# pananananas/MVD

Hardware: AMD Instinct MI355X
Metric: UNet forward-passes/sec @512x512 SD2.1+MV adapter (higher is better)
Workload: dtype bf16; 1 GPU; cfg4: configs[3]/[4]: 8 objects x 4 target views per GPU (32 pairs), camera FiLM + cross-view adapter; pairs_per_gpu=32, global_pairs=32, latent=64x64x4, image=512x512, forward=cold, hip_graph=False, q2_statistics=replica-local, parallelism=dp1 (pairs sharded by object), weights=synthetic seeded, SD2.1 shapes (865.9M UNet x2 + 99.2M adapter + 19.1M camera), encoder_weights=distinct

## Files before the change

### include/mvd_hip.h

```cpp
#ifndef MVD_HIP_H
#define MVD_HIP_H
#include <stddef.h>
#include <stdint.h>

#ifdef __cplusplus
extern "C" {
#endif

#define MVD_MAX_LEVELS 4

typedef struct {
  int in_channels;
  int out_channels;
  int num_levels;
  int block_out_channels[MVD_MAX_LEVELS];
  int num_heads[MVD_MAX_LEVELS];
  int layers_per_block;
  int cross_attention_dim;
  int norm_num_groups;
  float norm_eps;
  int cam_output_dim;
  int cam_hidden_dim;
  int simple_cam_encoder;
  float cam_modulation_strength;
// ... 66 lines not shown
                  int ld_rowvec, int rows_per_batch, const void* res, float alpha, int geglu, void* out, int out_f32,
                  int m, int n, int force_cfg, int splitk, float* splitk_ws ,
                  void* stream);
int mvd_op_ln_linear(const void* x, int k, const void* w_folded, const float* c1, const float* c2, float eps, int geglu,
                     void* out, int m, int n, void* stream);
int mvd_op_linear_xs(const void* x, int ldx, const void* w_packed, int m, int k, int units, int geglu, int ln, float ln_eps,
                     const void* res, int ldres, void* out, int ldo, int csplit, void* stream);
int mvd_op_conv3x3_ws(const void* x, int batch, int h, int w, int c, const void* w_packed, const float* bias, const float* rowvec,
                      int ld_rowvec, const void* res, const void* sc, const void* sc2, int sc_c1, int sc_c2, void* out, int n,
                      int variant, void* stream);
int mvd_op_conv3x3(const void* x, int batch, int in_h, int in_w, int cin, int stride, int upsample, int asym_pad, const void* w,
                   const float* bias, const float* rowvec, int ld_rowvec, const void* res, const void* sc, const void* sc2,
                   int sc_c1, int sc_c2, void* out, int cout, int force_cfg, int splitk, float* splitk_ws, void* stream);
int mvd_op_conv3x3_up4(const void* x, int batch, int in_h, int in_w, int cin, const void* w4, const float* bias, void* out, int cout,
                       int force_cfg, void* stream);
int mvd_op_attention(const void* q, const void* k, const void* v, void* o, int batch, int heads, int nq, int nk, int ldq,
                     int ldk, int ldv, int ldo, float scale, void* stream);
int64_t mvd_op_attention_split_ws_bytes(int batch, int heads, int nq, int nsplit);
int mvd_op_attention_split(const void* q, const void* k, const void* v, void* o, int batch, int heads, int nq, int nk, int ldq,
                           int ldk, int ldv, int ldo, int nsplit, void* ws, void* stream);
int mvd_op_groupnorm(const void* x0, const void* x1, int c0, int c1, int batch, int hw, int groups, float eps,
                     const float* gamma, const float* beta, int silu, void* y, float* ws, void* stream);
int mvd_op_layernorm(const void* x, int rows, int c, float eps, const float* gamma, const float* beta, void* y,
                     void* stream);
int mvd_op_refnorm(const void* x, int batch, int hw, int c, void* y, void* stream);
int mvd_op_film(const void* x, int batch, int hw, int c, const float* scale, const float* shift, void* y, void* stream);
int mvd_op_conv_in(const void* x, int batch, int h, int w, int cin, const float* wt, const float* bias, int cout, void* y,
                   void* stream);
int mvd_op_conv_out(const void* x, int batch, int h, int w, int c, const void* wt, const float* bias, int cout, float* y,
                    void* stream);
// ... 154 lines not shown
```

### mvd_amd/_lib.py

```python
from __future__ import annotations

import ctypes as C
import enum
import os

HERE = os.path.dirname(os.path.abspath(__file__))
LIB_PATH = os.environ.get("MVD_HIP_LIB") or os.path.join(HERE, "libmvd_hip.so")

MVD_MAX_LEVELS = 4
MVD_USE_CAMERA, MVD_USE_IMAGE, MVD_REUSE_REF, MVD_KEEP_FEATURES = 1, 2, 4, 8


class MvdError(RuntimeError):
    pass


class DebugFlag(enum.IntFlag):
    NO_SM_LN_FOLD = 1
    SM_NO_SPLITK = 2
    NO_SM = 4
    NO_SPLIT_KV = 8
    ONE_STREAM = 16
    SINGLE_STREAM_POLICY = 32
    SIDE_DEFAULT_PRIORITY = 64
# ... 105 lines not shown
    "mvd_op_layernorm": (C.c_int, [C.c_void_p, C.c_int, C.c_int, C.c_float, C.c_void_p, C.c_void_p, C.c_void_p, C.c_void_p]),
    "mvd_op_refnorm": (C.c_int, [C.c_void_p, C.c_int, C.c_int, C.c_int, C.c_void_p, C.c_void_p]),
    "mvd_op_film": (C.c_int, [C.c_void_p, C.c_int, C.c_int, C.c_int, C.c_void_p, C.c_void_p, C.c_void_p, C.c_void_p]),
    "mvd_op_conv_in": (C.c_int, [C.c_void_p, C.c_int, C.c_int, C.c_int, C.c_int, C.c_void_p, C.c_void_p, C.c_int, C.c_void_p, C.c_void_p]),
    "mvd_op_conv_out": (C.c_int, [C.c_void_p, C.c_int, C.c_int, C.c_int, C.c_int, C.c_void_p, C.c_void_p, C.c_int, C.c_void_p, C.c_void_p]),
    "mvd_op_nchw_to_nhwc": (C.c_int, [C.c_void_p, C.c_int, C.c_int, C.c_int, C.c_void_p, C.c_void_p, C.c_void_p, C.c_void_p]),
    "mvd_op_nhwc_to_nchw": (C.c_int, [C.c_void_p, C.c_int, C.c_int, C.c_int, C.c_void_p, C.c_void_p]),
    "mvd_op_f32_to_bf16": (C.c_int, [C.c_void_p, C.c_int64, C.c_void_p, C.c_void_p]),
    "mvd_op_skinny_linear": (C.c_int, [C.c_void_p, C.c_int, C.c_int, C.c_int, C.c_void_p, C.c_int, C.c_void_p, C.c_int, C.c_int,
                                        C.c_void_p, C.c_int, C.c_void_p]),
    "mvd_gemm_num_configs": (C.c_int, []),
    "mvd_debug_last_gemm_plan": (C.c_int, [C.POINTER(C.c_int)]),
    "mvd_debug_up4_launches": (C.c_long, []),
    "mvd_op_conv3x3_up4": (C.c_int, [C.c_void_p, C.c_int, C.c_int, C.c_int, C.c_int, C.c_void_p, C.c_void_p, C.c_void_p, C.c_int, C.c_int,
                                     C.c_void_p]),
    "mvd_debug_last_gemm_nowait": (C.c_int, []),
    "mvd_debug_last_attention_plan": (C.c_int, [C.POINTER(C.c_int)]),
    "mvd_debug_pick_splitk": (C.c_int, [C.c_int, C.c_int, C.c_int, C.c_int]),
    "mvd_debug_pick_splitk_conv": (C.c_int, [C.c_int, C.c_int, C.c_int]),
    "mvd_gemm_sm_num_tiles": (C.c_int, []),
    "mvd_debug_set_attention_nw": (C.c_int, [C.c_int]),
    "mvd_debug_set_flags": (C.c_int, [C.c_int]),
    "mvd_op_ddpm_step": (C.c_int, [C.c_void_p, C.c_void_p, C.c_void_p, C.c_float, C.c_float, C.c_float, C.c_float,
                                   C.c_float, C.c_void_p, C.c_int64, C.c_void_p]),
    "mvd_op_cfg_combine": (C.c_int, [C.c_void_p, C.c_float, C.c_void_p, C.c_int64, C.c_void_p]),
    "mvd_op_sampler_step": (C.c_int, [C.c_void_p, C.c_int, C.c_float, C.c_void_p, C.c_void_p, C.c_void_p, C.c_float, C.c_float,
                                      C.c_float, C.c_float, C.c_float, C.c_float, C.c_void_p, C.c_void_p, C.c_int64, C.c_void_p]),
    "mvd_op_add_noise": (C.c_int, [C.c_void_p, C.c_void_p, C.c_void_p, C.c_void_p, C.c_void_p, C.c_int, C.c_void_p, C.c_void_p, C.c_int,
                                   C.c_int64, C.c_void_p]),
    "mvd_op_noise_loss_ws_bytes": (C.c_int64, [C.c_int, C.c_int64]),
# ... 91 lines not shown
```

### mvd_amd/csrc/engine.hip

```cpp
#include <math.h>
#include <stdio.h>
#include <stdlib.h>
#include <string.h>

#include <string>
#include <unordered_map>
#include <vector>

#include "host_util.h"

int mvd_launch_silu_to_bf16(const float* x, int64_t n, bf16_t* y, hipStream_t s);

static int g_debug_flags = 0;
extern "C" int mvd_debug_set_flags(int flags) { g_debug_flags = flags; return 0; }
int mvd_debug_flags() { return g_debug_flags; }

namespace {

struct FeatureInfo { std::string name; int level; int C; int heads; std::string key;  };
constexpr int MVD_REF_ONLY_INTERNAL = 1 << 30;

}

struct mvd_engine {
// ... 310 lines not shown
        g_debug_flags = saved;
        g_ws_ptrs[0] = (const char*)x.p; g_ws_lens[0] = (size_t)x.rows() * x.C * 2;
        g_ws_ptrs[1] = (const char*)sc0; g_ws_lens[1] = (size_t)out.rows() * scc0 * 2;
        g_ws_ptrs[2] = (const char*)sc1; g_ws_lens[2] = (size_t)out.rows() * scc1 * 2;
        g_ws_ptrs[3] = (const char*)out.p; g_ws_lens[3] = (size_t)out.rows() * out.C * 2;
        ws_check_launch(slot, set, nowait, out.p, chk.p, (long)out.rows() * out.C, s);
      }
      e->tmp.off = mark;
    }
#endif
    return r ? r : 1;
  }

  int conv3(const Act& x, int stride, int ups, const bf16_t* w, const float* bias, const float* rowvec, int ld_rowvec,
            const bf16_t* res, const bf16_t* sc0, const bf16_t* sc1, int scc0, int scc1, Act& out, const std::string& ws = std::string(),
            const std::string& w4 = std::string()) {
    if (!ws.empty() && stride == 1) {
      const int r = try_ws(x, ups, ws, bias, rowvec, ld_rowvec, res, sc0, sc1, scc0, scc1, out);
      if (r) return r < 0 ? r : 0;
    }
    MvdGemmArgs g = gemm_conv3(x.p, x.H, x.W, x.C, stride, ups, 0, sc0, sc1, scc0, scc1, w, bias, out.B, out.H, out.W, out.C, out.p);
    g.rowvec = rowvec; g.ld_rowvec = ld_rowvec; g.res = res;
    if (!w4.empty() && !dry && !err && ups == 1 && stride == 1 && !sc0 && !res && !rowvec && !(g_debug_flags & MVD_DBG_NO_UP4) && has(w4)) {
      int t_ = 0, n_ = 0, s_ = 1, S = 1, fc = -1;
      if (!(sm_enabled() && mvd_gemm_sm_plan(g, &t_, &n_, &s_))) {
        tiled_plan(g, S, fc);
        MvdGemmArgs u = g;
        u.splitk = 1;
        if (S == 1 && (fc >= 0 ? fc : mvd_gemm_pick_config(u)) == 7 && mvd_gemm_pp_applicable(u)) {
          gemm_conv3_to_up4(u);
          if (mvd_gemm_pp_up4_applicable(u)) {
            u.W = WB(w4, (int64_t)4 * out.C * 4 * x.C);
            if (!u.W) return err;
            e->prof_M = u.M; e->prof_N = u.N; e->prof_K = u.Ktot; e->prof_tag = 140;
            return profiled(MVD_PC_PP_CONV3, 2.0 * u.M * (double)u.N * u.Ktot, 0.0, [&] { return mvd_launch_gemm(u, s, 7); });
          }
        }
      }
    }
    return gemm(g);
  }

  int groupnorm(const bf16_t* x0, const bf16_t* x1, int c0, int c1, int B, int hw, float eps, const float* g, const float* b,
                int silu, bf16_t* y) {
    if (err) return err;
    const int groups = e->cfg.norm_num_groups;
// ... 249 lines not shown
      if (!o.capture && i >= o.late_from) c.e->dual_late = true;
      for (int j = 0; j <= Lb; ++j) {
        Act skip = skips.back(); skips.pop_back();
        if (skip.H != h.H || skip.W != h.W) { mvd_set_error("up block %d: skip %dx%d vs hidden %dx%d (odd latent size unsupported)", i, skip.H, skip.W, h.H, h.W); return -13; }
        Act r = c.new_act(B, h.H, h.W, co, true);
        CHECK(resnet(bk + ".resnets." + std::to_string(j), h, &skip, co, r));
        h = r;
        if (i > 0) {
          Act t = c.new_act(B, h.H, h.W, co, true);
          CHECK(transformer(bk + ".attentions." + std::to_string(j), h, cfg.num_heads[n - 1 - i], t));
          h = t;
        }
      }
      if (i + 1 < n) {
        Act u = c.new_act(B, h.H * 2, h.W * 2, co, true);
        CHECK(c.conv3(h, 1, 1, c.WB(bk + ".up.w", (int64_t)co * 9 * co), c.WF(bk + ".up.b", co), nullptr, 0, nullptr, nullptr, nullptr, 0, 0, u, bk + ".up.ws", bk + ".up.w4"));
        h = u;
      }
      if (o.film) { Act res = h; CHECK(film("up_" + std::to_string(i), h, res)); h = res; }
    }
    if (out_nchw) {
      Act t = c.new_act(B, h.H, h.W, C0, false);
      CHECK(c.groupnorm(h.p, nullptr, C0, 0, B, h.hw(), cfg.norm_eps, c.WF("conv_norm_out.g", C0), c.WF("conv_norm_out.b", C0), 1, t.p));
      const bf16_t* wo = c.WB("conv_out.w", (int64_t)cfg.out_channels * 9 * C0);
      const float* bo = c.WF("conv_out.b", cfg.out_channels);
      if (!c.dry && !c.err) CHECK(mvd_launch_conv_out(t.p, B, h.H, h.W, C0, wo, bo, cfg.out_channels, out_nchw, c.s));
    }
    return c.err;
  }
};

int time_path(Ctx& c, const float* timesteps, int B, const float** tproj_out) {
// ... 660 lines not shown
                             (const bf16_t*)w, bias, batch, oh, ow, cout, out);
  g.rowvec = rowvec; g.ld_rowvec = ld_rowvec; g.res = (const bf16_t*)res;
  return op_launch(g, force_cfg, splitk, splitk_ws, (hipStream_t)stream);
}

int mvd_op_conv3x3_up4(const void* x, int batch, int in_h, int in_w, int cin, const void* w4, const float* bias, void* out, int cout,
                       int force_cfg, void* stream) {
  if (!x || !w4 || !out || batch <= 0 || in_h <= 0 || in_w <= 0 || cin <= 0 || cout <= 0) { mvd_set_error("mvd_op_conv3x3_up4: bad argument"); return -1; }
  MvdGemmArgs g = gemm_conv3((const bf16_t*)x, in_h, in_w, cin, 1, 1, 0, nullptr, nullptr, 0, 0, (const bf16_t*)w4, bias, batch, 2 * in_h, 2 * in_w,
                             cout, out);
  gemm_conv3_to_up4(g);
  g.splitk = 1;
  return mvd_launch_gemm(g, (hipStream_t)stream, force_cfg);
}

int mvd_op_attention(const void* q, const void* k, const void* v, void* o, int batch, int heads, int nq, int nk, int ldq,
                     int ldk, int ldv, int ldo, float scale, void* stream) {
  MvdAttnArgs a; memset(&a, 0, sizeof(a));
  a.nprob = 1; a.batch = batch; a.heads = heads; a.scale = scale;
  a.prescaled = scale == 0.f;
  a.p[0] = {(const bf16_t*)q, (const bf16_t*)k, (const bf16_t*)v, (bf16_t*)o, ldq, ldk, ldv, ldo,
            (int64_t)nq * ldq, (int64_t)nk * ldk, (int64_t)nk * ldv, (int64_t)nq * ldo, nq, nk};
  return mvd_launch_attention(a, (hipStream_t)stream);
}

int64_t mvd_op_attention_split_ws_bytes(int batch, int heads, int nq, int nsplit) {
  MvdAttnArgs a; memset(&a, 0, sizeof(a));
  a.nprob = 1; a.batch = batch; a.heads = heads; a.p[0].nq = nq;
  return (int64_t)mvd_attention_split_ws_bytes(a, nsplit) + (int64_t)mvd_attention_split_counters(a) * 4 + 256;
}
// ... 50 lines not shown
```

### mvd_amd/csrc/gemm.hip

```cpp
#include <stdlib.h>
#include <string.h>
#include "kernels.h"
#include "gemm_tile.h"

thread_local MvdLaunchPlan g_mvd_last_gemm = {-1, 1, 0, 0, 0, 0};

namespace {

__global__ __launch_bounds__(256) void splitk_reduce_kernel(const MvdGemmArgs a) {
  const long nvec = (long)a.M * (a.N >> 2);
  const int nv = a.N >> 2;
  for (long e = (long)blockIdx.x * blockDim.x + threadIdx.x; e < nvec; e += (long)gridDim.x * blockDim.x) {
    const int m = (int)(e / nv), n = (int)(e - (long)m * nv) * 4;
    f32x4 v = *reinterpret_cast<const f32x4*>(a.part + (size_t)m * a.N + n);
    for (int s = 1; s < a.splitk; ++s) v += *reinterpret_cast<const f32x4*>(a.part + ((size_t)s * a.M + m) * a.N + n);
    if (a.bias) v += *reinterpret_cast<const f32x4*>(a.bias + n);
    if (a.rowvec) v += *reinterpret_cast<const f32x4*>(a.rowvec + (size_t)(m / a.rows_per_batch) * a.ld_rowvec + n);
    v *= a.alpha;
    if (a.res) {
      const u32x2 r = *reinterpret_cast<const u32x2*>(a.res + (size_t)m * a.ldres + n);
      v[0] += bflo(r[0]); v[1] += bfhi(r[0]); v[2] += bflo(r[1]); v[3] += bfhi(r[1]);
    }
    if (a.out_f32) {
      *reinterpret_cast<f32x4*>(reinterpret_cast<float*>(a.out) + (size_t)m * a.ldo + n) = v;
// ... 111 lines not shown
    ksum += g.ksize;
  }
  if (a.nseg == 2 && !(a.seg[0].mode == MVD_A_CONV3 && a.seg[1].mode == MVD_A_DENSE)) { mvd_set_error("gemm: a second segment must be a dense segment after a conv segment"); return -1; }
  if (ksum != a.Ktot) { mvd_set_error("gemm: segment K sum %d != Ktot %d", ksum, a.Ktot); return -1; }
  if (a.ldw < a.Ktot || (a.ldw % 8) || !a.W) { mvd_set_error("gemm: bad weight stride ldw=%d (K=%d)", a.ldw, a.Ktot); return -1; }
  if (a.rows_per_batch <= 0) { mvd_set_error("gemm: rows_per_batch must be > 0"); return -1; }
  if (a.N % 64) { mvd_set_error("gemm: N=%d must be a multiple of 64", a.N); return -1; }
  if (a.splitk > 1 && (!a.part || a.geglu || a.splitk > (force_cfg >= 100 ? 64 : 16) || a.splitk > a.Ktot / 64)) { mvd_set_error("gemm: bad split-K request (splitk=%d)", a.splitk); return -1; }
  if (a.geglu && (a.out_f32 || a.res || a.rowvec)) { mvd_set_error("gemm: unsupported GEGLU epilogue combination"); return -1; }
  if (a.relu && (a.relu != 1 || a.geglu || a.ln_c1 || a.nseg != 1 || a.w_blocked || (a.seg[0].mode == MVD_A_CONV3 && a.seg[0].ups == 2))) {
    mvd_set_error("gemm: the ReLU epilogue takes one dense or one 3x3 segment (no GEGLU, LayerNorm fold, fused shortcut, sub-pixel upsampler, blocked weights)");
    return -1;
  }
  const int on = a.geglu ? a.N / 2 : a.N;
  if (a.ldo < on || (a.ldo % 4) || (a.res && (a.ldres % 4))) { mvd_set_error("gemm: bad leading dims"); return -1; }

  static const int default_glds = MVD_ENV_INT("MVD_GEMM_GLDS", 1);
  bool glds = default_glds != 0;
#ifdef MVD_PROBE
  static const int dbg = MVD_ENV_INT("MVD_GEMM_DEBUG", 0);
  if (dbg) const_cast<MvdGemmArgs&>(a).dbg = dbg;
#endif
  if (a.seg[0].mode == MVD_A_CONV3 && a.seg[0].ups == 2) {
    if ((force_cfg >= 0 && force_cfg != 7) || (a.dbg & ~32) || !mvd_gemm_pp_up4_applicable(a)) {
      mvd_set_error("gemm: the 2x2 sub-pixel upsampling convolution does not take this problem (in %dx%d C=%d N=%d cfg=%d): source width a multiple of 16 or 8 (even height), N %% 320 == 0, bias only, unsplit",
                    a.seg[0].inH, a.seg[0].inW, a.seg[0].c0, a.N, force_cfg);
      return -1;
    }
    g_mvd_last_gemm.cfg = 7; g_mvd_last_gemm.splitk = 1;
    return mvd_launch_gemm_pp(a, s);
// ... 97 lines not shown
```

### mvd_amd/csrc/gemm_pp.hip

```cpp
#include <stdlib.h>
#include <string.h>
#include "kernels.h"
#include "bufaddr.h"

namespace {

constexpr int BN = 320, NT = 512;
constexpr int B_BYTES = BN * 128, B_IT = BN * 8 / NT;

MVD_DEVINL int fresh_lane() {
  int l = (int)__builtin_amdgcn_mbcnt_hi(~0u, __builtin_amdgcn_mbcnt_lo(~0u, 0u));
  asm volatile("" : "+v"(l));
  return l;
}

MVD_DEVINL int swz_off(int row, int chunk) { return row * 128 + ((chunk ^ ((row >> 1) & 7)) << 4); }

constexpr int XCH_C1 = 0, XCH_C2 = 2048, XCH_STATS = 4096, XCH_BYTES = 6144;

template <int BM, int WM, int WN, int AMODE, bool SPLITK, bool LNF = false>
__global__ __launch_bounds__(NT, 2) void gemm_pp_kernel(const MvdGemmArgs a) {
  static_assert(!LNF || (AMODE == 0 && !SPLITK), "the LayerNorm fold is a dense, unsplit form");
  constexpr int A_BYTES = BM * 128, STAGE_BYTES = A_BYTES + B_BYTES;
  constexpr int A_IT = BM * 8 / NT;
  static_assert(A_IT == 4, "the A loader below is written for 256-row tiles");
  constexpr int WTM = BM / WM, WTN = BN / WN, TM = WTM / 16, TN = WTN / 16;
  constexpr bool GEGLU = WM == 4;
  constexpr bool HAS_CONV = AMODE != 0;
  constexpr bool UPS = AMODE == 3;
  constexpr bool UP4 = AMODE == 4;
  static_assert(!UP4 || !SPLITK, "the sub-pixel form is unsplit");
  static_assert((WTM * 128) % 2048 == 0 && (WTN % 16) == 0, "fragment rows of a wave share one swizzle pattern");
  extern __shared__ __attribute__((aligned(16))) unsigned char smem[];
  const int tid = threadIdx.x, lane = tid & 63;
  const int wave = __builtin_amdgcn_readfirstlane(tid >> 6);
  const int grp = wave >> 2;
  const int wm = wave / WN, wn = wave % WN;
  const int ntn = a.N / BN;
  const int srcM = UP4 ? a.M >> 2 : a.M;
  const int ntm = (srcM + BM - 1) / BM;
  const int lrow = tid >> 3;
  const int kc = (tid & 7) ^ ((lrow >> 1) & 7);
  const int w4 = wave & 3;
  const int arow = w4 * 8 + (lane >> 3);

// ... 312 lines not shown
    } else {
      const bool has_res = !UP4 && a.res != nullptr;
      unsigned up_b = 0, up_y = 0, up_x = 0;
      if constexpr (UP4) {
        const unsigned hw = (unsigned)(cs.inH * cs.inW);
        up_b = (unsigned)row0 / hw;
        const unsigned rem = (unsigned)row0 - up_b * hw;
        up_y = rem / (unsigned)cs.inW; up_x = rem - up_y * (unsigned)cs.inW;
      }
      __amdgpu_buffer_rsrc_t rs_r = rs_o;
      if (has_res) rs_r = buf_rsrc(a.res, (int)((size_t)a.M * a.ldres * 2));
      const int vr16 = (fr * a.ldres + pair_col) * 2, vr8 = (fr * a.ldres + fq * 4) * 2;
      constexpr int NP = TN / 2;
      f32x4 cb[TN];
      load_colconst(m0, n0, cb);
      const bool row_rv = a.rowvec && a.rows_per_batch % BM != 0;
      constexpr int RG = HAS_CONV ? 2 : 4;
#pragma unroll
      for (int i0 = 0; i0 < TM; i0 += RG) {
        u32x4 rp[RG][NP > 0 ? NP : 1];
        u32x2 rs1[RG];
        if (has_res) {
#pragma unroll
          for (int g = 0; g < RG; ++g) {
            const int so = ((row0 + (i0 + g) * 16) * a.ldres + n0 + wn * WTN) * 2;
#pragma unroll
            for (int q = 0; q < NP; ++q) rp[g][q] = __builtin_amdgcn_raw_buffer_load_b128(rs_r, vr16, so + q * 64, 0);
            if (TN & 1) rs1[g] = __builtin_amdgcn_raw_buffer_load_b64(rs_r, vr8, so + (TN - 1) * 32, 0);
          }
        }
#pragma unroll
        for (int g = 0; g < RG; ++g) {
          const int i = i0 + g;
          int so = ((row0 + i * 16) * a.ldo + n0 + wn * WTN) * 2;
          if constexpr (UP4) {
            const int orow = (int)((up_b * 2 * cs.inH + 2 * up_y + (up_par >> 1)) * a.outW + 2 * up_x + (up_par & 1));
            so = (row0 + i * 16 < srcM ? orow : a.M) * a.ldo * 2 + (n0 + wn * WTN) * 2;
            up_x += 16;
            if (up_x >= (unsigned)cs.inW) { up_x = 0; up_y += cs.inW >= 16 ? 1 : 2; }
            if (up_y >= (unsigned)cs.inH) { up_y = 0; ++up_b; }
          }
          int mrow = row0 + i * 16 + fr;
          mrow = mrow < a.M ? mrow : a.M - 1;
          const float* rvp = row_rv ? a.rowvec + (size_t)(mrow / a.rows_per_batch) * a.ld_rowvec + n0 + wn * WTN + fq * 4 : nullptr;
          auto finish = [&](f32x4 v, int j, u32x2 r) -> u32x2 {
            v += cb[j];
            if (row_rv) v += *reinterpret_cast<const f32x4*>(rvp + j * 16);
            v *= alpha;
            if (has_res) { v[0] += bflo(r[0]); v[1] += bfhi(r[0]); v[2] += bflo(r[1]); v[3] += bfhi(r[1]); }
            return u32x2{pack2bf(v[0], v[1]), pack2bf(v[2], v[3])};
          };
#pragma unroll
          for (int q = 0; q < NP; ++q) {
            u32x2 ra = {0u, 0u}, rb = {0u, 0u};
            if (has_res) {
              ra = u32x2{rp[g][q][0], rp[g][q][1]}; rb = u32x2{rp[g][q][2], rp[g][q][3]};
              swap_pair(ra, rb);
            }
            u32x2 oa = finish(acc[i][2 * q], 2 * q, ra), ob = finish(acc[i][2 * q + 1], 2 * q + 1, rb);
            swap_pair(oa, ob);
            store16(u32x4{oa[0], oa[1], ob[0], ob[1]}, rs_o, vo16, so + q * 64);
          }
          if (TN & 1) __builtin_amdgcn_raw_buffer_store_b64(finish(acc[i][TN - 1], TN - 1, has_res ? rs1[g] : u32x2{0u, 0u}), rs_o, vo8, so + (TN - 1) * 32, 0);
        }
// ... 134 lines not shown
  if (grp == 0) phase_end();
}

template <int BM, int WM, int WN, int AMODE, bool SPLITK, bool LNF = false>
int launch_pp(const MvdGemmArgs& a, hipStream_t s) {
  constexpr int LDS_BYTES = 2 * (BM * 128 + B_BYTES) + (LNF ? XCH_BYTES : 0);
  static bool init[16] = {};
  int dev = 0;
  (void)hipGetDevice(&dev);
  if (!init[dev & 15]) {
    hipError_t e = hipFuncSetAttribute(reinterpret_cast<const void*>(&gemm_pp_kernel<BM, WM, WN, AMODE, SPLITK, LNF>),
                                       hipFuncAttributeMaxDynamicSharedMemorySize, LDS_BYTES);
    if (e != hipSuccess) { mvd_set_error("gemm_pp: hipFuncSetAttribute: %s", hipGetErrorString(e)); return -2; }
    init[dev & 15] = true;
  }
  const int ntm = ((AMODE == 4 ? a.M / 4 : a.M) + BM - 1) / BM, ntn = a.N / BN;
  MvdGemmArgs b = a;
  b.walk_cg = SPLITK ? 0 : mvd_gemm_pp_walk(a);
  int grid = 256;
  const int ntiles = ntm * ntn * (a.splitk > 1 ? a.splitk : 1) * (AMODE == 4 ? 4 : 1);
  if (ntiles < grid) grid = ((ntiles + 7) / 8) * 8;
  g_mvd_last_gemm.tiles = ntiles; g_mvd_last_gemm.grid = grid; g_mvd_last_gemm.per_cu = 1;
  hipLaunchKernelGGL((gemm_pp_kernel<BM, WM, WN, AMODE, SPLITK, LNF>), dim3(grid), dim3(NT), LDS_BYTES, s, b);
  hipError_t e = hipGetLastError();
  if (e != hipSuccess) { mvd_set_error("gemm_pp launch: %s", hipGetErrorString(e)); return -3; }
  return 0;
}

template <int BM, int WM, int WN>
int launch_pp_mode(const MvdGemmArgs& a, hipStream_t s) {
  const bool sk = a.splitk > 1;
  if (a.seg[0].mode == MVD_A_DENSE) return sk ? launch_pp<BM, WM, WN, 0, true>(a, s) : launch_pp<BM, WM, WN, 0, false>(a, s);
  if (a.seg[0].ups == 2) {
    if (!mvd_gemm_pp_up4_applicable(a)) { mvd_set_error("gemm_pp: not a problem of the 2x2 sub-pixel upsampling convolution"); return -1; }
    g_mvd_up4_launches.fetch_add(1);
    return launch_pp<BM, WM, WN, 4, false>(a, s);
  }
  if (a.seg[0].ups) {
    if (a.nseg != 1) { mvd_set_error("gemm_pp: an upsampling convolution takes no shortcut segment"); return -1; }
    return sk ? launch_pp<BM, WM, WN, 3, true>(a, s) : launch_pp<BM, WM, WN, 3, false>(a, s);
  }
  if (a.nseg == 1) return sk ? launch_pp<BM, WM, WN, 1, true>(a, s) : launch_pp<BM, WM, WN, 1, false>(a, s);
  return sk ? launch_pp<BM, WM, WN, 2, true>(a, s) : launch_pp<BM, WM, WN, 2, false>(a, s);
}

}

int mvd_gemm_pp_walk(const MvdGemmArgs& a) {
  static const int on = MVD_ENV_INT("MVD_GEMM_PP_WALK", 1);
  if (!on || (mvd_debug_flags() & MVD_DBG_PP_ROW_MAJOR) || a.walk_cg < 0) return 0;
  if (a.walk_cg > 0) return a.walk_cg;
// ... 25 lines not shown
      if (bytes + (size_t)3 * g.inW * g.c0 * 2 >= lim) return false;
      if (2 * g.inH >= 32768 || 2 * g.inW >= 32768) return false;
    }
  }
  return true;
}

bool mvd_gemm_pp_up4_applicable(const MvdGemmArgs& a) {
  const MvdASeg& g = a.seg[0];
  if (a.nseg != 1 || g.mode != MVD_A_CONV3 || g.ups != 2 || g.stride != 1 || g.asym || g.c1) return false;
  if (a.res || a.rowvec || a.splitk > 1 || a.geglu || a.ln_c1 || a.out_f32) return false;
  if (g.c0 <= 0 || g.c0 % 64 || g.ksize != 4 * g.c0 || a.Ktot != 4 * g.c0 || a.ldw != a.Ktot) return false;
  if (g.inH <= 0 || g.inW <= 0 || a.outH != 2 * g.inH || a.outW != 2 * g.inW || a.rows_per_batch != a.outH * a.outW || a.M % a.rows_per_batch) return false;
  if (!(g.inW % 16 == 0 || (g.inW == 8 && g.inH % 2 == 0))) return false;
  const size_t lim = (size_t)1 << 31;
  if ((size_t)4 * a.N * a.ldw * 2 >= lim) return false;
  if ((size_t)(a.M + 2 * a.outW + 16 + 256) * a.ldo * 2 >= lim) return false;
  return mvd_gemm_pp_applicable(a);
}

int mvd_launch_gemm_pp(const MvdGemmArgs& a, hipStream_t s) {
  if (a.ln_c1) {
    const MvdASeg& g = a.seg[0];
    if (a.nseg != 1 || g.mode != MVD_A_DENSE || g.c1 || a.splitk > 1 || a.res || a.rowvec || !a.bias) {
      mvd_set_error("gemm_pp: the LayerNorm fold takes one dense source, a bias, no residual / row vector / split-K"); return -1;
    }
    return a.geglu ? launch_pp<256, 4, 2, 0, false, true>(a, s) : launch_pp<256, 2, 4, 0, false, true>(a, s);
  }
  if (a.geglu) {
    if (a.seg[0].mode != MVD_A_DENSE || a.splitk > 1) { mvd_set_error("gemm_pp: GEGLU needs a dense, unsplit problem"); return -1; }
// ... 14 lines not shown
```

### mvd_amd/csrc/gemm_sm.hip

```cpp
#include <stdlib.h>
#include <string.h>
#include "kernels.h"
#include "bufaddr.h"

namespace {

template <int N> MVD_DEVINL void wait_vm() { asm volatile("s_waitcnt vmcnt(%0)" ::"n"(N) : "memory"); }
template <int L> MVD_DEVINL void wait_groups(int ahead) {
  constexpr int C1 = L > 63 ? 63 : L, C2 = 2 * L > 63 ? 63 : 2 * L, C3 = 3 * L > 63 ? 63 : 3 * L, C4 = 4 * L > 63 ? 63 : 4 * L,
                C5 = 5 * L > 63 ? 63 : 5 * L, C6 = 6 * L > 63 ? 63 : 6 * L;
  switch (ahead) {
    case 0: wait_vm<0>(); break;
    case 1: wait_vm<C1>(); break;
    case 2: wait_vm<C2>(); break;
    case 3: wait_vm<C3>(); break;
    case 4: wait_vm<C4>(); break;
    case 5: wait_vm<C5>(); break;
    default: wait_vm<C6>(); break;
  }
}

constexpr int SM_MAX_STAGES = 8;

template <int BM, int BN, int AMODE, bool SPLITK, bool GEGLU, bool LNF = false>
// ... 414 lines not shown
    else { mvd_set_error("gemm_sm: GEGLU needs an even number of 16-column tiles per wave"); return -1; }
  }
  if (a.ln_c1) return launch_sm3<BM, BN, 0, false, false, true>(a, nstage, s);
  if (a.seg[0].mode == MVD_A_DENSE) return sk ? launch_sm3<BM, BN, 0, true, false>(a, nstage, s) : launch_sm3<BM, BN, 0, false, false>(a, nstage, s);
  if (a.nseg == 1) return sk ? launch_sm3<BM, BN, 1, true, false>(a, nstage, s) : launch_sm3<BM, BN, 1, false, false>(a, nstage, s);
  return sk ? launch_sm3<BM, BN, 2, true, false>(a, nstage, s) : launch_sm3<BM, BN, 2, false, false>(a, nstage, s);
}

}

bool mvd_gemm_sm_applicable(const MvdGemmArgs& a, int tile) {
  if (tile < 0 || tile >= kNumSmTiles) return false;
  const size_t lim = (size_t)1 << 31;
  if (a.N % kSmTiles[tile].bn || a.Ktot % 64) return false;
  if (a.relu) return false;
  if (a.ln_c1) {
    const MvdASeg& g = a.seg[0];
    if (a.nseg != 1 || g.mode != MVD_A_DENSE || g.c1 || a.splitk > 1 || a.res || a.rowvec || a.out_f32 || !a.bias || a.Ktot != g.c0) return false;
  }
  if (a.w_blocked && a.ldw != a.Ktot) return false;
  if (a.geglu && ((kSmTiles[tile].bn / 32) % 2 || a.splitk > 1 || a.seg[0].mode != MVD_A_DENSE)) return false;
  if ((size_t)a.N * a.ldw * 2 >= lim) return false;
  if (a.splitk > 1 && ((size_t)a.splitk * a.M * a.N * 4 >= lim || !a.tile_cnt || !a.part || a.splitk > 24)) return false;
  for (int i = 0; i < a.nseg; ++i) {
    const MvdASeg& g = a.seg[i];
    if (g.mode == MVD_A_DENSE) {
      if ((size_t)a.M * (g.c0 > g.c1 ? g.c0 : g.c1) * 2 >= lim) return false;
    } else {
      const size_t bytes = (size_t)(a.M / a.rows_per_batch) * g.inH * g.inW * g.c0 * 2 + (size_t)(g.inW + 1) * g.c0 * 2;
      if (bytes + (size_t)3 * g.inW * g.c0 * 2 >= lim) return false;
// ... 58 lines not shown
```

### mvd_amd/csrc/kernels.h

```cpp
#pragma once
#include <hip/hip_runtime.h>
#include <stdint.h>
#include <atomic>
#include "common.h"
#include "../../include/mvd_hip.h"

enum { MVD_A_DENSE = 0, MVD_A_CONV3 = 1 };

struct MvdASeg {
  const bf16_t* p0;
  const bf16_t* p1;
  int c0, c1;
  int mode;
  int ksize;
  int inH, inW;
  int stride;
  int ups;
  int asym;
};

struct MvdGemmArgs {
  MvdASeg seg[2];
  int nseg;
  const bf16_t* W;
// ... 9 lines not shown
  float alpha;
  int geglu;
  void* out;
  int ldo;
  int out_f32;
  int splitk;
  float* part;
  int w_blocked;
  int splitk_nowait;
  unsigned int* tile_cnt;
  int dbg;
  int relu;
  const float* ln_c1;
  float ln_eps;
  int walk_cg;
};
static_assert(sizeof(MvdGemmArgs) == 280, "MvdGemmArgs is a kernel argument: a size change moves the hidden arguments of every GEMM kernel");

int mvd_launch_gemm(const MvdGemmArgs& a, hipStream_t s, int force_cfg = -1);
int mvd_gemm_pick_config(const MvdGemmArgs& a);
int mvd_launch_gemm_relu(const MvdGemmArgs& a, hipStream_t s, int cfg, bool glds);
int mvd_launch_splitk_reduce_relu(const MvdGemmArgs& a, hipStream_t s, int grid);
struct MvdLaunchPlan { int cfg, splitk, tiles, grid, per_cu, nowait; };
extern thread_local MvdLaunchPlan g_mvd_last_gemm;
extern std::atomic<long> g_mvd_up4_launches;
bool mvd_gemm_pp_applicable(const MvdGemmArgs& a);
bool mvd_gemm_pp_up4_applicable(const MvdGemmArgs& a);
int mvd_gemm_pp_walk(const MvdGemmArgs& a);
int mvd_debug_flags();
bool mvd_gemm_ln_fold_ok(const MvdGemmArgs& a);
int mvd_launch_gemm_pp(const MvdGemmArgs& a, hipStream_t s);
int mvd_launch_gemm_ring(const MvdGemmArgs& a, hipStream_t s);
// ... 117 lines not shown
```

### mvd_amd/csrc/misc.hip

```cpp
#include <stdarg.h>
#include <stdio.h>
#include <stdlib.h>
#include "kernels.h"

static thread_local char g_err[512] = "";
void mvd_set_error(const char* fmt, ...) {
  va_list ap;
  va_start(ap, fmt);
  vsnprintf(g_err, sizeof(g_err), fmt, ap);
  va_end(ap);
}
extern "C" const char* mvd_last_error(void) { return g_err; }

namespace {

__global__ void nchw_to_nhwc_kernel(const float* __restrict__ x, int c, int hw, const float* __restrict__ scale,
                                    const float* __restrict__ shift, int ld_ss, bf16_t* __restrict__ y, long total) {
  const long i = (long)blockIdx.x * blockDim.x + threadIdx.x;
  if (i >= total) return;
  const int ch = i % c;
  const long bp = i / c;
  const int p = bp % hw;
  const int b = bp / hw;
  float v = x[((size_t)b * c + ch) * hw + p];
// ... 82 lines not shown
        float a = acc[co];
#pragma unroll
        for (int j = 0; j < 4; ++j) {
          a = fmaf(bflo(xv[j]), bflo(wv[j]), a);
          a = fmaf(bfhi(xv[j]), bfhi(wv[j]), a);
        }
        acc[co] = a;
      }
    }
  }
#pragma unroll
  for (int co = 0; co < 8; ++co) {
    if (co < cout) {
      const float t = wave_sum(acc[co]);
      if (lane == 0) y[((size_t)b * cout + co) * hw + p] = t + bias[co];
    }
  }
}

__global__ void f32_to_bf16_kernel(const float* __restrict__ x, long n, bf16_t* __restrict__ y) {
  for (long i = (long)blockIdx.x * blockDim.x + threadIdx.x; i < n; i += (long)gridDim.x * blockDim.x) y[i] = f2bf(x[i]);
}

template <bool WBF16>
__global__ __launch_bounds__(256) void skinny_linear_kernel(const float* __restrict__ x, int ldx, int batch, int k,
                                                             const void* __restrict__ wv, const float* __restrict__ bias,
                                                             int n, int act_in, float* __restrict__ y, int ldy) {
  constexpr int BC = 32;
  const int lane = threadIdx.x & 63;
  const int o = blockIdx.x * 4 + (threadIdx.x >> 6);
// ... 361 lines not shown
      hipLaunchKernelGGL(conv_out_kernel, dim3(nblk((long)batch * h * w, 4)), dim3(256), 0, s, x, batch, h, w, c, wt, bias, cout, yr);
      hipLaunchKernelGGL(conv_out_cmp_kernel, dim3(256), dim3(256), 0, s, y, yb, yr, (long)on, 1e-3f, cnt);
      ++calls;
      volatile unsigned long long* vc = cnt;
      const unsigned long long c0 = vc[0], c1 = vc[1], c2 = vc[2];
      if (c0 != seen[0] || c1 != seen[1] || c2 != seen[2] || calls == 2 || calls == 20) {
        seen[0] = c0; seen[1] = c1; seen[2] = c2;
        fprintf(stderr, "conv_out cmp pid %d after ~%d calls: first!=second %llu  |first-ref|>1e-3 %llu  |second-ref|>1e-3 %llu  last idx %llu (x mod 4 = %llu)\n",
                (int)getpid(), calls - 1, c0, c1, c2, (unsigned long long)vc[3], (unsigned long long)vc[3] % 4);
      }
    }
    return check("conv_out4");
  }
#endif
  const long pix = (long)batch * h * w;
  hipLaunchKernelGGL(conv_out_kernel, dim3(nblk(pix, 4)), dim3(256), 0, s, x, batch, h, w, c, wt, bias, cout, y);
  return check("conv_out");
}

int mvd_launch_f32_to_bf16(const float* x, int64_t n, bf16_t* y, hipStream_t s) {
  if (!x || !y || n <= 0) { mvd_set_error("f32_to_bf16: bad arguments"); return -1; }
  int grid = nblk(n, 256);
  if (grid > 4096) grid = 4096;
  hipLaunchKernelGGL(f32_to_bf16_kernel, dim3(grid), dim3(256), 0, s, x, (long)n, y);
  return check("f32_to_bf16");
}

int mvd_launch_skinny_linear(const float* x, int ldx, int batch, int k, const void* w, int wbf16, const float* bias, int n,
                             int act_in, float* y, int ldy, hipStream_t s) {
  if (!x || !w || !y || batch <= 0 || batch > 4096 || k <= 0 || n <= 0 || ldx < k || ldy < n) { mvd_set_error("skinny_linear: bad arguments"); return -1; }
// ... 108 lines not shown
```

### mvd_amd/ops.py

```python
from __future__ import annotations

import ctypes as C
from typing import Optional

import torch

from . import _lib as L


def _p(t: Optional[torch.Tensor]):
    if t is None:
        return None
    assert t.is_cuda and t.is_contiguous(), "ops expect contiguous CUDA tensors"
    return C.c_void_p(t.data_ptr())


def _s():
    return C.c_void_p(torch.cuda.current_stream().cuda_stream)


def _bf16(*ts):
    for t in ts:
        if t is not None:
            assert t.dtype == torch.bfloat16, "expected bf16"
# ... 74 lines not shown
    c2 = shortcut2.shape[-1] if shortcut2 is not None else 0
    ws = torch.empty(splitk * B * oh * ow * cout + 4096, device=x.device, dtype=torch.float32) if splitk > 1 else None
    L.call("mvd_op_conv3x3", _p(x), B, H, W, Cin, stride, int(upsample), int(asym_pad), _p(w_packed), _p(bias), _p(rowvec),
           rowvec.shape[1] if rowvec is not None else 0, _p(res), _p(shortcut), _p(shortcut2), c1, c2, _p(out), cout,
           force_cfg, splitk, _p(ws), _s())
    return out


def conv3x3_up4(x, w4, bias=None, force_cfg=-1):
    _bf16(x, w4)
    B, H, W, Cin = x.shape
    assert w4.dim() == 3 and w4.shape[0] == 4 and w4.shape[2] == 4 * Cin and w4.is_contiguous() and x.is_contiguous(), tuple(w4.shape)
    cout = w4.shape[1]
    out = torch.empty(B, 2 * H, 2 * W, cout, device=x.device, dtype=torch.bfloat16)
    L.call("mvd_op_conv3x3_up4", _p(x), B, H, W, Cin, _p(w4), _p(bias), _p(out), cout, force_cfg, _s())
    return out


def conv3x3_relu(x, w_packed, bias=None, relu=True, out_f32=False, force_cfg=-1, splitk=1):
    _bf16(x, w_packed)
    B, H, W, Cin = x.shape
    cout = w_packed.shape[0]
    assert w_packed.shape[1] == 9 * Cin, (tuple(w_packed.shape), Cin)
    out = torch.empty(B, H, W, cout, device=x.device, dtype=torch.float32 if out_f32 else torch.bfloat16)
    ws = torch.empty(splitk * B * H * W * cout, device=x.device, dtype=torch.float32) if splitk > 1 else None
    L.call("mvd_op_conv3x3_relu", _p(x), B, H, W, Cin, _p(w_packed), _p(bias), _p(out), cout, int(relu), int(out_f32), force_cfg,
           splitk, _p(ws), _s())
    return out


# ... 272 lines not shown
```

Measured before the change: 539.8 forward-passes/s.

## Fuse FiLM into up-sampling conv epilogue and add MFMA conv_out kernel

Adds a FiLM (per-batch scale/shift) epilogue to the 2x2 sub-pixel upsampling conv GEMM, so the decoder upsample blocks no longer launch a separate film kernel that re-reads and re-writes the upsampled activation. The GEMM argument struct grows by three fields, and new guards keep FiLM out of other GEMM paths. Separately, conv_out gets an MFMA-based kernel for channel counts divisible by 32, replacing the scalar wave-reduction path. The risks are a larger kernel argument block for every GEMM and extra per-element buffer loads in the epilogue.

```diff
diff --git a/include/mvd_hip.h b/include/mvd_hip.h
--- a/include/mvd_hip.h
+++ b/include/mvd_hip.h
@@ -104,6 +104,8 @@
                    int sc_c1, int sc_c2, void* out, int cout, int force_cfg, int splitk, float* splitk_ws, void* stream);
 int mvd_op_conv3x3_up4(const void* x, int batch, int in_h, int in_w, int cin, const void* w4, const float* bias, void* out, int cout,
                        int force_cfg, void* stream);
+int mvd_op_conv3x3_up4_film(const void* x, int batch, int in_h, int in_w, int cin, const void* w4, const float* bias, const float* scale,
+                            const float* shift, void* out, int cout, void* stream);
 int mvd_op_attention(const void* q, const void* k, const void* v, void* o, int batch, int heads, int nq, int nk, int ldq,
                      int ldk, int ldv, int ldo, float scale, void* stream);
 int64_t mvd_op_attention_split_ws_bytes(int batch, int heads, int nq, int nsplit);
diff --git a/mvd_amd/_lib.py b/mvd_amd/_lib.py
--- a/mvd_amd/_lib.py
+++ b/mvd_amd/_lib.py
@@ -143,6 +143,8 @@
     "mvd_debug_up4_launches": (C.c_long, []),
     "mvd_op_conv3x3_up4": (C.c_int, [C.c_void_p, C.c_int, C.c_int, C.c_int, C.c_int, C.c_void_p, C.c_void_p, C.c_void_p, C.c_int, C.c_int,
                                      C.c_void_p]),
+    "mvd_op_conv3x3_up4_film": (C.c_int, [C.c_void_p, C.c_int, C.c_int, C.c_int, C.c_int, C.c_void_p, C.c_void_p, C.c_void_p, C.c_void_p, C.c_void_p,
+                                          C.c_int, C.c_void_p]),
     "mvd_debug_last_gemm_nowait": (C.c_int, []),
     "mvd_debug_last_attention_plan": (C.c_int, [C.POINTER(C.c_int)]),
     "mvd_debug_pick_splitk": (C.c_int, [C.c_int, C.c_int, C.c_int, C.c_int]),
diff --git a/mvd_amd/csrc/engine.hip b/mvd_amd/csrc/engine.hip
--- a/mvd_amd/csrc/engine.hip
+++ b/mvd_amd/csrc/engine.hip
@@ -348,7 +348,7 @@
 
   int conv3(const Act& x, int stride, int ups, const bf16_t* w, const float* bias, const float* rowvec, int ld_rowvec,
             const bf16_t* res, const bf16_t* sc0, const bf16_t* sc1, int scc0, int scc1, Act& out, const std::string& ws = std::string(),
-            const std::string& w4 = std::string()) {
+            const std::string& w4 = std::string(), const float* film_sc = nullptr, const float* film_sh = nullptr, bool* filmed = nullptr) {
     if (!ws.empty() && stride == 1) {
       const int r = try_ws(x, ups, ws, bias, rowvec, ld_rowvec, res, sc0, sc1, scc0, scc1, out);
       if (r) return r < 0 ? r : 0;
@@ -363,7 +363,13 @@
         u.splitk = 1;
         if (S == 1 && (fc >= 0 ? fc : mvd_gemm_pick_config(u)) == 7 && mvd_gemm_pp_applicable(u)) {
           gemm_conv3_to_up4(u);
+          const bool fold = film_sc && film_sh && filmed;
+          if (fold) {
+            u.film_scale = film_sc; u.film_shift = film_sh; u.ld_film = out.C;
+            if (!mvd_gemm_pp_up4_applicable(u)) { u.film_scale = u.film_shift = nullptr; u.ld_film = 0; }
+          }
           if (mvd_gemm_pp_up4_applicable(u)) {
+            if (u.film_scale) *filmed = true;
             u.W = WB(w4, (int64_t)4 * out.C * 4 * x.C);
             if (!u.W) return err;
             e->prof_M = u.M; e->prof_N = u.N; e->prof_K = u.Ktot; e->prof_tag = 140;
@@ -643,8 +649,16 @@
       }
       if (i + 1 < n) {
         Act u = c.new_act(B, h.H * 2, h.W * 2, co, true);
-        CHECK(c.conv3(h, 1, 1, c.WB(bk + ".up.w", (int64_t)co * 9 * co), c.WF(bk + ".up.b", co), nullptr, 0, nullptr, nullptr, nullptr, 0, 0, u, bk + ".up.ws", bk + ".up.w4"));
+        const float *fsc = nullptr, *fsh = nullptr;
+        bool filmed = false;
+        if (o.film) {
+          auto it = o.film_ss->find("up_" + std::to_string(i));
+          if (it != o.film_ss->end()) { fsc = it->second.first; fsh = it->second.second; }
+        }
+        CHECK(c.conv3(h, 1, 1, c.WB(bk + ".up.w", (int64_t)co * 9 * co), c.WF(bk + ".up.b", co), nullptr, 0, nullptr, nullptr, nullptr, 0, 0, u, bk + ".up.ws", bk + ".up.w4",
+                      fsc, fsh, &filmed));
         h = u;
+        if (filmed) continue;
       }
       if (o.film) { Act res = h; CHECK(film("up_" + std::to_string(i), h, res)); h = res; }
     }
@@ -1335,6 +1349,17 @@
   return mvd_launch_gemm(g, (hipStream_t)stream, force_cfg);
 }
 
+int mvd_op_conv3x3_up4_film(const void* x, int batch, int in_h, int in_w, int cin, const void* w4, const float* bias, const float* scale,
+                            const float* shift, void* out, int cout, void* stream) {
+  if (!x || !w4 || !out || !scale || !shift || batch <= 0 || in_h <= 0 || in_w <= 0 || cin <= 0 || cout <= 0) { mvd_set_error("mvd_op_conv3x3_up4_film: bad argument"); return -1; }
+  MvdGemmArgs g = gemm_conv3((const bf16_t*)x, in_h, in_w, cin, 1, 1, 0, nullptr, nullptr, 0, 0, (const bf16_t*)w4, bias, batch, 2 * in_h, 2 * in_w,
+                             cout, out);
+  gemm_conv3_to_up4(g);
+  g.splitk = 1;
+  g.film_scale = scale; g.film_shift = shift; g.ld_film = cout;
+  return mvd_launch_gemm(g, (hipStream_t)stream, 7);
+}
+
 int mvd_op_attention(const void* q, const void* k, const void* v, void* o, int batch, int heads, int nq, int nk, int ldq,
                      int ldk, int ldv, int ldo, float scale, void* stream) {
   MvdAttnArgs a; memset(&a, 0, sizeof(a));
diff --git a/mvd_amd/csrc/gemm.hip b/mvd_amd/csrc/gemm.hip
--- a/mvd_amd/csrc/gemm.hip
+++ b/mvd_amd/csrc/gemm.hip
@@ -149,6 +149,10 @@
   }
   const int on = a.geglu ? a.N / 2 : a.N;
   if (a.ldo < on || (a.ldo % 4) || (a.res && (a.ldres % 4))) { mvd_set_error("gemm: bad leading dims"); return -1; }
+  if ((a.film_scale || a.film_shift) && !(a.seg[0].mode == MVD_A_CONV3 && a.seg[0].ups == 2)) {
+    mvd_set_error("gemm: the FiLM epilogue exists in the 2x2 sub-pixel upsampling convolution only (callers keep film_kernel elsewhere)");
+    return -1;
+  }
 
   static const int default_glds = MVD_ENV_INT("MVD_GEMM_GLDS", 1);
   bool glds = default_glds != 0;
diff --git a/mvd_amd/csrc/gemm_pp.hip b/mvd_amd/csrc/gemm_pp.hip
--- a/mvd_amd/csrc/gemm_pp.hip
+++ b/mvd_amd/csrc/gemm_pp.hip
@@ -28,7 +28,8 @@
   constexpr bool GEGLU = WM == 4;
   constexpr bool HAS_CONV = AMODE != 0;
   constexpr bool UPS = AMODE == 3;
-  constexpr bool UP4 = AMODE == 4;
+  constexpr bool UP4 = AMODE == 4 || AMODE == 5;
+  constexpr bool FILM = AMODE == 5;
   static_assert(!UP4 || !SPLITK, "the sub-pixel form is unsplit");
   static_assert((WTM * 128) % 2048 == 0 && (WTN % 16) == 0, "fragment rows of a wave share one swizzle pattern");
   extern __shared__ __attribute__((aligned(16))) unsigned char smem[];
@@ -371,6 +372,11 @@
       constexpr int NP = TN / 2;
       f32x4 cb[TN];
       load_colconst(m0, n0, cb);
+      __amdgpu_buffer_rsrc_t rs_fs = rs_o, rs_ft = rs_o;
+      if constexpr (FILM) {
+        const int fbytes = (a.M / a.rows_per_batch) * a.ld_film * 4;
+        rs_fs = buf_rsrc(a.film_scale, fbytes); rs_ft = buf_rsrc(a.film_shift, fbytes);
+      }
       const bool row_rv = a.rowvec && a.rows_per_batch % BM != 0;
       constexpr int RG = HAS_CONV ? 2 : 4;
 #pragma unroll
@@ -390,7 +396,9 @@
         for (int g = 0; g < RG; ++g) {
           const int i = i0 + g;
           int so = ((row0 + i * 16) * a.ldo + n0 + wn * WTN) * 2;
+          int so_film = 0;
           if constexpr (UP4) {
+            if constexpr (FILM) so_film = ((int)up_b * a.ld_film + n0 + wn * WTN) * 4;
             const int orow = (int)((up_b * 2 * cs.inH + 2 * up_y + (up_par >> 1)) * a.outW + 2 * up_x + (up_par & 1));
             so = (row0 + i * 16 < srcM ? orow : a.M) * a.ldo * 2 + (n0 + wn * WTN) * 2;
             up_x += 16;
@@ -405,6 +413,12 @@
             if (row_rv) v += *reinterpret_cast<const f32x4*>(rvp + j * 16);
             v *= alpha;
             if (has_res) { v[0] += bflo(r[0]); v[1] += bfhi(r[0]); v[2] += bflo(r[1]); v[3] += bfhi(r[1]); }
+            if constexpr (FILM) {
+              const f32x4 sc = __builtin_bit_cast(f32x4, __builtin_amdgcn_raw_buffer_load_b128(rs_fs, fq * 16, so_film + j * 64, 0));
+              const f32x4 sh = __builtin_bit_cast(f32x4, __builtin_amdgcn_raw_buffer_load_b128(rs_ft, fq * 16, so_film + j * 64, 0));
+#pragma unroll
+              for (int e = 0; e < 4; ++e) v[e] = fmaf(v[e], sc[e], sh[e]);
+            }
             return u32x2{pack2bf(v[0], v[1]), pack2bf(v[2], v[3])};
           };
 #pragma unroll
@@ -569,11 +583,11 @@
     if (e != hipSuccess) { mvd_set_error("gemm_pp: hipFuncSetAttribute: %s", hipGetErrorString(e)); return -2; }
     init[dev & 15] = true;
   }
-  const int ntm = ((AMODE == 4 ? a.M / 4 : a.M) + BM - 1) / BM, ntn = a.N / BN;
+  const int ntm = ((AMODE >= 4 ? a.M / 4 : a.M) + BM - 1) / BM, ntn = a.N / BN;
   MvdGemmArgs b = a;
   b.walk_cg = SPLITK ? 0 : mvd_gemm_pp_walk(a);
   int grid = 256;
-  const int ntiles = ntm * ntn * (a.splitk > 1 ? a.splitk : 1) * (AMODE == 4 ? 4 : 1);
+  const int ntiles = ntm * ntn * (a.splitk > 1 ? a.splitk : 1) * (AMODE >= 4 ? 4 : 1);
   if (ntiles < grid) grid = ((ntiles + 7) / 8) * 8;
   g_mvd_last_gemm.tiles = ntiles; g_mvd_last_gemm.grid = grid; g_mvd_last_gemm.per_cu = 1;
   hipLaunchKernelGGL((gemm_pp_kernel<BM, WM, WN, AMODE, SPLITK, LNF>), dim3(grid), dim3(NT), LDS_BYTES, s, b);
@@ -589,7 +603,7 @@
   if (a.seg[0].ups == 2) {
     if (!mvd_gemm_pp_up4_applicable(a)) { mvd_set_error("gemm_pp: not a problem of the 2x2 sub-pixel upsampling convolution"); return -1; }
     g_mvd_up4_launches.fetch_add(1);
-    return launch_pp<BM, WM, WN, 4, false>(a, s);
+    return a.film_scale ? launch_pp<BM, WM, WN, 5, false>(a, s) : launch_pp<BM, WM, WN, 4, false>(a, s);
   }
   if (a.seg[0].ups) {
     if (a.nseg != 1) { mvd_set_error("gemm_pp: an upsampling convolution takes no shortcut segment"); return -1; }
@@ -645,6 +659,10 @@
   if (g.inH <= 0 || g.inW <= 0 || a.outH != 2 * g.inH || a.outW != 2 * g.inW || a.rows_per_batch != a.outH * a.outW || a.M % a.rows_per_batch) return false;
   if (!(g.inW % 16 == 0 || (g.inW == 8 && g.inH % 2 == 0))) return false;
   const size_t lim = (size_t)1 << 31;
+  if (a.film_scale || a.film_shift) {
+    if (!a.film_scale || !a.film_shift || a.ld_film < a.N || (a.ld_film & 3) || (((uintptr_t)a.film_scale | (uintptr_t)a.film_shift) & 15)) return false;
+    if ((size_t)(a.M / a.rows_per_batch + 2) * a.ld_film * 4 >= lim) return false;
+  }
   if ((size_t)4 * a.N * a.ldw * 2 >= lim) return false;
   if ((size_t)(a.M + 2 * a.outW + 16 + 256) * a.ldo * 2 >= lim) return false;
   return mvd_gemm_pp_applicable(a);
diff --git a/mvd_amd/csrc/gemm_sm.hip b/mvd_amd/csrc/gemm_sm.hip
--- a/mvd_amd/csrc/gemm_sm.hip
+++ b/mvd_amd/csrc/gemm_sm.hip
@@ -452,6 +452,7 @@
   const size_t lim = (size_t)1 << 31;
   if (a.N % kSmTiles[tile].bn || a.Ktot % 64) return false;
   if (a.relu) return false;
+  if (a.film_scale || a.film_shift) return false;
   if (a.ln_c1) {
     const MvdASeg& g = a.seg[0];
     if (a.nseg != 1 || g.mode != MVD_A_DENSE || g.c1 || a.splitk > 1 || a.res || a.rowvec || a.out_f32 || !a.bias || a.Ktot != g.c0) return false;
diff --git a/mvd_amd/csrc/kernels.h b/mvd_amd/csrc/kernels.h
--- a/mvd_amd/csrc/kernels.h
+++ b/mvd_amd/csrc/kernels.h
@@ -47,8 +47,11 @@
   const float* ln_c1;
   float ln_eps;
   int walk_cg;
+  const float* film_scale;
+  const float* film_shift;
+  int ld_film;
 };
-static_assert(sizeof(MvdGemmArgs) == 280, "MvdGemmArgs is a kernel argument: a size change moves the hidden arguments of every GEMM kernel");
+static_assert(sizeof(MvdGemmArgs) == 304, "MvdGemmArgs is a kernel argument: a size change moves the hidden arguments of every GEMM kernel");
 
 int mvd_launch_gemm(const MvdGemmArgs& a, hipStream_t s, int force_cfg = -1);
 int mvd_gemm_pick_config(const MvdGemmArgs& a);
diff --git a/mvd_amd/csrc/misc.hip b/mvd_amd/csrc/misc.hip
--- a/mvd_amd/csrc/misc.hip
+++ b/mvd_amd/csrc/misc.hip
@@ -2,6 +2,7 @@
 #include <stdio.h>
 #include <stdlib.h>
 #include "kernels.h"
+#include "bufaddr.h"
 
 static thread_local char g_err[512] = "";
 void mvd_set_error(const char* fmt, ...) {
@@ -120,6 +121,63 @@
     if (co < cout) {
       const float t = wave_sum(acc[co]);
       if (lane == 0) y[((size_t)b * cout + co) * hw + p] = t + bias[co];
+    }
+  }
+}
+
+template <int U>
+__global__ __launch_bounds__(256) void conv_out_mfma_kernel(const bf16_t* __restrict__ x, int batch, int h, int w, int c,
+                                                             const bf16_t* __restrict__ wt, const float* __restrict__ bias,
+                                                             int cout, float* __restrict__ y) {
+  const int lane = threadIdx.x & 63, n = lane & 15, g = lane >> 4;
+  const int segs = (w + 31) >> 5;
+  const long unit = (long)blockIdx.x * 4 + (threadIdx.x >> 6);
+  if (unit >= (long)batch * h * segs) return;
+  const int seg = unit % segs;
+  const long by = unit / segs;
+  const int oy = by % h, b = by / h;
+  const int ox0 = seg * 32 + n;
+  const __amdgpu_buffer_rsrc_t rs_x = buf_rsrc(x, (unsigned)((size_t)batch * h * w * c * 2));
+  const __amdgpu_buffer_rsrc_t rs_w = buf_rsrc(wt, (unsigned)((size_t)cout * 9 * c * 2));
+  const int ks = c >> 5;
+  f32x4 acc[2] = {{0.f, 0.f, 0.f, 0.f}, {0.f, 0.f, 0.f, 0.f}};
+  for (int tap = 0; tap < 9; ++tap) {
+    const int iy = oy + tap / 3 - 1, dx = tap % 3 - 1;
+    unsigned vx[2];
+#pragma unroll
+    for (int t = 0; t < 2; ++t) {
+      const int ox = ox0 + 16 * t, ix = ox + dx;
+      const bool in = (unsigned)iy < (unsigned)h && (unsigned)ix < (unsigned)w && ox < w;
+      vx[t] = in ? ((unsigned)((b * h + iy) * w + ix) * c + 8 * g) * 2u : OOB;
+    }
+    const unsigned vw = n < cout ? (unsigned)(((n * 9 + tap) * c + 8 * g) * 2) : OOB;
+    for (int s0 = 0; s0 < ks; s0 += U) {
+      u32x4 xf[U][2], wf[U];
+#pragma unroll
+      for (int u = 0; u < U; ++u) {
+        const int so = (s0 + u) * 64;
+        wf[u] = __builtin_amdgcn_raw_buffer_load_b128(rs_w, (int)vw + so, 0, 0);
+        xf[u][0] = __builtin_amdgcn_raw_buffer_load_b128(rs_x, (int)vx[0] + so, 0, 0);
+        xf[u][1] = __builtin_amdgcn_raw_buffer_load_b128(rs_x, (int)vx[1] + so, 0, 0);
+      }
+#pragma unroll
+      for (int u = 0; u < U; ++u) {
+        const bf16x8 a = __builtin_bit_cast(bf16x8, wf[u]);
+        acc[0] = __builtin_amdgcn_mfma_f32_16x16x32_bf16(a, __builtin_bit_cast(bf16x8, xf[u][0]), acc[0], 0, 0, 0);
+        acc[1] = __builtin_amdgcn_mfma_f32_16x16x32_bf16(a, __builtin_bit_cast(bf16x8, xf[u][1]), acc[1], 0, 0, 0);
+      }
+    }
+  }
+  const size_t hw = (size_t)h * w;
+#pragma unroll
+  for (int i = 0; i < 4; ++i) {
+    const int co = 4 * g + i;
+    if (co >= cout) continue;
+    const float bv = bias[co];
+#pragma unroll
+    for (int t = 0; t < 2; ++t) {
+      const int ox = ox0 + 16 * t;
+      if (ox < w) y[((size_t)b * cout + co) * hw + (size_t)oy * w + ox] = acc[t][i] + bv;
     }
   }
 }
@@ -511,6 +569,13 @@
   }
 #endif
   const long pix = (long)batch * h * w;
+  if (c % 32 == 0 && (size_t)pix * c * 2 <= (size_t)OOB) {
+    const long units = (long)batch * h * ((w + 31) / 32);
+    const int ks = c / 32;
+    auto* k = ks % 5 == 0 ? conv_out_mfma_kernel<5> : ks % 4 == 0 ? conv_out_mfma_kernel<4> : ks % 2 == 0 ? conv_out_mfma_kernel<2> : conv_out_mfma_kernel<1>;
+    hipLaunchKernelGGL(k, dim3(nblk(units, 4)), dim3(256), 0, s, x, batch, h, w, c, wt, bias, cout, y);
+    return check("conv_out_mfma");
+  }
   hipLaunchKernelGGL(conv_out_kernel, dim3(nblk(pix, 4)), dim3(256), 0, s, x, batch, h, w, c, wt, bias, cout, y);
   return check("conv_out");
 }
diff --git a/mvd_amd/ops.py b/mvd_amd/ops.py
--- a/mvd_amd/ops.py
+++ b/mvd_amd/ops.py
@@ -112,6 +112,18 @@
     cout = w4.shape[1]
     out = torch.empty(B, 2 * H, 2 * W, cout, device=x.device, dtype=torch.bfloat16)
     L.call("mvd_op_conv3x3_up4", _p(x), B, H, W, Cin, _p(w4), _p(bias), _p(out), cout, force_cfg, _s())
+    return out
+
+
+def conv3x3_up4_film(x, w4, bias, scale, shift):
+    _bf16(x, w4)
+    B, H, W, Cin = x.shape
+    assert w4.dim() == 3 and w4.shape[0] == 4 and w4.shape[2] == 4 * Cin and w4.is_contiguous() and x.is_contiguous(), tuple(w4.shape)
+    cout = w4.shape[1]
+    assert scale.shape == (B, cout) and shift.shape == (B, cout) and scale.dtype == shift.dtype == torch.float32
+    assert scale.is_contiguous() and shift.is_contiguous()
+    out = torch.empty(B, 2 * H, 2 * W, cout, device=x.device, dtype=torch.bfloat16)
+    L.call("mvd_op_conv3x3_up4_film", _p(x), B, H, W, Cin, _p(w4), _p(bias), _p(scale), _p(shift), _p(out), cout, _s())
     return out
 
 
```

After: 541.1 forward-passes/s (median of 6 runs). Within noise of the previous version (+0.3%).
